# HKUST-Aerial-Robotics/Omni-swarm

Hardware: NVIDIA H100
Metric: keyframes/sec (SuperPoint+NetVLAD+match) (higher is better)
Workload: dtype f32

## Files before the change

omni-swarm_b200/csrc/kernels.cuh:

```cuda
#pragma once
#include "common.cuh"

namespace osb {

int db_scan_grid(int64_t n, int64_t* chunk_out);
osb_status db_search_device(const void* rows, int storage, int64_t n, const int64_t* n_dev, int dim, const float* q_dev,
                            int nq, int k, float* part_scores, int64_t* part_ids, unsigned int* done, float* scores_dev,
                            int64_t* ids_dev, cudaStream_t st);
osb_status db_rows_alloc(Resources& m, void** rows, size_t n, int storage);
osb_status db_rows_to_half(__half* dst, const float* src, size_t n, cudaStream_t st);
osb_status bf_match_device(int n_pairs, int max_n, int out_stride, const float* const* q, const int32_t* nq,
                           const float* const* t,
                           const int32_t* nt, float* dist_scratch, int32_t* qi, int32_t* ti, float* dout,
                           int32_t* n_out, int32_t* map_out, cudaStream_t st, int group = 0, size_t group_stride = 0);

enum Act { ACT_NONE = 0, ACT_RELU = 1, ACT_RELU6 = 2 };

struct ConvLayer {
  int cin = 0, cout = 0, cout_pad = 0, ks = 1;
  float* w = nullptr;
  float* b = nullptr;
};
osb_status conv_layer_upload(Resources& res, ConvLayer* L, const float* w_oihw, const float* bias, int cin, int cout, int ks);
osb_status upload_tap_major(Resources& res, float** dst, const float* w_oihw, int cout);

osb_status conv_forward(const ConvLayer& L, const float* x, float* y, int B, int H, int W, int out_cstride,
                        int act, cudaStream_t st);
osb_status conv_first_forward(const float* w_tap_cout , const float* bias, const float* lut,
                              const uint8_t* img, float* y, int B, int H, int W, int cout, int stride, int act,
                              cudaStream_t st);
osb_status maxpool2x2_forward(const float* x, float* y, int B, int H, int W, int C, cudaStream_t st);
osb_status dwconv3x3_forward(const float* w_tap_c, const float* bias, const float* x, float* y, int B, int H, int W,
                             int C, int stride, int act, cudaStream_t st);

osb_status sp_softmax_shuffle(const float* logits, int cstride, float* semi, int B, int Hc, int Wc, cudaStream_t st);
osb_status l2norm_cells(float* x, int64_t cells, int C, cudaStream_t st);

struct KeypointScratch {
  uint8_t* state = nullptr;
  uint8_t* surv = nullptr;
  int32_t* cand = nullptr;
  unsigned long long* skey = nullptr;
  unsigned long long* cmask = nullptr;
  bool write_surv = true;
  int32_t* counts = nullptr;
  float* cnorm = nullptr;
};
osb_status sp_keypoints(const float* semi, int B, int H, int W, float thres, int max_num, KeypointScratch& ks,
                        int32_t* n_kpts, float* kpts, float* conf, cudaStream_t st);
osb_status sp_descriptors(const float* desc_nhwc, int B, int H, int W, const int32_t* n_kpts, const float* kpts,
                          int max_num, const float* pca_compT , const float* pca_mean, float* cnorm, float* out,
                          cudaStream_t st);
osb_status nchw_to_nhwc(const float* in, float* out, int B, int C, int h, int w, cudaStream_t st);
osb_status nhwc_to_nchw(const float* in, float* out, int B, int C, int h, int w, cudaStream_t st);

osb_status stereo_lift_device(const float* kp_up, const float* kp_down, const int32_t* match, const int32_t* n_up,
                              const int32_t* n_down, int n_dirs, int max_n, const double* K, const double* pose_up,
                              const double* pose_down, double triangle_thres, int min_pts, float* pts3d, uint8_t* flag_up,
                              uint8_t* flag_down, cudaStream_t st, bool down_main = false);
osb_status depth_lift_device(const float* kp, const int32_t* n_kp, int n_dirs, int max_n, const uint16_t* depth_mm, int H,
                             int W, const double* K, const double* pose_cam, double near_thres, double far_thres,
                             int min_pts, float* pts3d, uint8_t* flag, cudaStream_t st);
osb_status homography_ransac_device(const float* src_dev, const float* dst_dev, const int32_t* n_dev, int n_pairs, int max_n,
                                    float thresh, uint32_t seed, uint8_t* mask_dev, int32_t* n_inl_dev, int32_t* winner_dev,
                                    cudaStream_t st, unsigned int* scratch );

constexpr int PNP_THREADS = 256;
constexpr int PNP_MAXN = 1024;
__global__ void __launch_bounds__(PNP_THREADS)
pnp_ransac_kernel(const float* __restrict__ pts3d, const float* __restrict__ pts2d, const int32_t* __restrict__ n_pts, int max_n,
                  const osb_pnp_params* __restrict__ params, uint8_t* __restrict__ mask_out, osb_pnp_result* __restrict__ results);

}
```

omni-swarm_b200/csrc/keyframe.cu:

```cuda
#include "superpoint.cuh"
#include "pose_algebra.cuh"
#include <atomic>

namespace osb {

struct DbDev {
  int64_t ntotal;
  int nframes;
};

struct FeFeedback {
  volatile long long seq_begin;
  volatile long long n_local, n_remote, charged;
  volatile long long seq_end;
};

struct DbView {
  DbDev* dev;
  int storage;
  void* rows;
  float* ldesc;
  float* kpts;
  int32_t* lflag;
  int32_t* nk;
// ... 722 lines not shown
  OSB_TRY(m.alloc(&g.g_mask, sk));
  OSB_TRY(m.alloc(&g.g_keys, 2 * (size_t)slots));
  OSB_CUDA(cudaMemsetAsync(g.g_keys, 0, 2 * (size_t)slots * sizeof(unsigned int), st));
  return OSB_OK;
}

extern "C" osb_status osb_frontend_create(osb_frontend** out, const osb_frontend_config* cfg, const float* sp_weights,
                                          size_t n_sp_weights, const float* pca_comp, const float* pca_mean,
                                          const float* nv_weights, size_t n_nv_weights) {
  OSB_REQUIRE(out && cfg && sp_weights && pca_comp && pca_mean && nv_weights, "null argument");
  OSB_REQUIRE(cfg->n_dirs >= 1 && cfg->n_dirs <= OSB_MAX_DIRS, "n_dirs must be 1..4");
  OSB_REQUIRE(cfg->max_num >= 1 && cfg->max_num <= OSB_MAX_KPTS, "max_num must be 1..200");
  OSB_REQUIRE(cfg->query_dir >= 0 && cfg->query_dir < cfg->n_dirs, "query_dir out of range");
  OSB_REQUIRE(cfg->db_capacity > 0 && cfg->db_capacity < (1 << 30), "bad db_capacity");
  OSB_REQUIRE(cfg->match_index_dist >= 1 && 5 + cfg->match_index_dist <= FE_KMAX, "bad match_index_dist");
  OSB_TRY(require_device());
  std::unique_ptr<osb_frontend> h(new osb_frontend());
  h->cfg = *cfg;
  h->device = current_device();
  const int nd = cfg->n_dirs, mn = cfg->max_num;
  Resources& m = h->res;
  OSB_TRY(m.stream(&h->stream));
  OSB_TRY(m.stream(&h->stream2));
  OSB_TRY(m.event(&h->ev_fork, cudaEventDisableTiming));
  OSB_TRY(m.event(&h->ev_join, cudaEventDisableTiming));
  OSB_TRY(m.event(&h->ev_ingest, cudaEventDisableTiming));
  OSB_TRY(m.host_alloc(&h->h_cnt, 2, cudaHostAllocDefault));
  OSB_TRY(m.host_alloc(&h->fb_host, 1, cudaHostAllocMapped));
  memset((void*)h->fb_host, 0, sizeof(FeFeedback));
  OSB_CUDA(cudaHostGetDevicePointer((void**)&h->fb_dev, (void*)h->fb_host, 0));
  OSB_TRY(h->sp.init(sp_weights, n_sp_weights, cfg->width, cfg->height, cfg->sp_thres, mn, pca_comp, pca_mean, 2 * nd));
  h->sp.ks.write_surv = false;
  if (cfg->zero_bottom_quarter) OSB_TRY(h->sp.band_init());
  OSB_TRY(h->nv.init(nv_weights, n_nv_weights, cfg->width, cfg->height, nd));
  OSB_TRY(dbstore_alloc(m, h->db[0], cfg->db_capacity, mn));
  OSB_TRY(dbstore_alloc(m, h->db[1], cfg->db_capacity, mn));
  const size_t HW = (size_t)cfg->width * cfg->height, dk = (size_t)OSB_MAX_DIRS * OSB_MAX_KPTS, dm = (size_t)OSB_MAX_DIRS * mn;
  OSB_TRY(m.alloc(&h->d_img, 2 * nd * HW));
  OSB_TRY(m.alloc(&h->d_st_pairs, 1));
  OSB_TRY(m.alloc(&h->d_q_pairs, 1));
  OSB_TRY(m.alloc(&h->d_st_qi, dm));
  OSB_TRY(m.alloc(&h->d_st_ti, dm));
  OSB_TRY(m.alloc(&h->d_st_map, dm));
  OSB_TRY(m.alloc(&h->d_st_n, OSB_MAX_DIRS));
  OSB_TRY(m.alloc(&h->d_st_dist, dm));
  OSB_TRY(m.alloc(&h->q1.dout, dk));
  OSB_TRY(fe_geo_alloc(m, h->q1, OSB_MAX_DIRS, 0));
  OSB_TRY(m.alloc(&h->d_dist_scratch, dm * mn));
  h->q1.pairs = fe_pair_view(h->d_q_pairs);
  h->q1.dist = h->d_dist_scratch;
  OSB_TRY(m.alloc(&h->d_assign, (size_t)h->max_records * OSB_MAX_DIRS));
  OSB_TRY(m.alloc(&h->d_cam_pose, 2 * OSB_MAX_DIRS * 7));
  OSB_TRY(m.alloc(&h->d_l3d, dm * 3));
  OSB_TRY(m.alloc(&h->d_lflag_up, dm));
  OSB_TRY(m.alloc(&h->d_lflag_down, dm));
  OSB_TRY(m.alloc(&h->d_record, 1));
  OSB_TRY(m.alloc(&h->d_result, 1));
  {
    FePairs st{};
    for (int d = 0; d < nd; ++d) {
      st.q[d] = h->sp.d_out + (size_t)d * mn * OSB_FEATURE_DESC_SIZE;
      st.t[d] = h->sp.d_out + (size_t)(nd + d) * mn * OSB_FEATURE_DESC_SIZE;
    }
    OSB_CUDA(cudaMemcpy(h->d_st_pairs, &st, sizeof(st), cudaMemcpyHostToDevice));
  }
  *out = h.release();
// ... 698 lines not shown
```

omni-swarm_b200/csrc/postproc.cu:

```cuda
#include "common.cuh"
#include "kernels.cuh"

namespace osb {

__global__ void sp_softmax_shuffle_kernel(const float* __restrict__ logits, int cstride, float* __restrict__ semi,
                                          int Hc, int Wc, int64_t cells) {
  const int64_t i = (int64_t)blockIdx.x * blockDim.x + threadIdx.x;
  if (i >= cells) return;
  const int cx = (int)(i % Wc);
  const int cy = (int)((i / Wc) % Hc);
  const int b = (int)(i / ((int64_t)Wc * Hc));
  const float* l = logits + (size_t)i * cstride;
  float v[65];
  float m = -INFINITY;
#pragma unroll
  for (int c = 0; c < 65; ++c) { v[c] = l[c]; m = fmaxf(m, v[c]); }
  float s = 0.f;
#pragma unroll
  for (int c = 0; c < 65; ++c) { v[c] = expf(v[c] - m); s += v[c]; }
  const int W = Wc * 8;
  float* out = semi + ((size_t)b * Hc * 8 + cy * 8) * W + cx * 8;
#pragma unroll
  for (int r = 0; r < 8; ++r) {
    float4 a = make_float4(v[r * 8 + 0] / s, v[r * 8 + 1] / s, v[r * 8 + 2] / s, v[r * 8 + 3] / s);
    float4 c = make_float4(v[r * 8 + 4] / s, v[r * 8 + 5] / s, v[r * 8 + 6] / s, v[r * 8 + 7] / s);
    reinterpret_cast<float4*>(out + (size_t)r * W)[0] = a;
    reinterpret_cast<float4*>(out + (size_t)r * W)[1] = c;
  }
}

osb_status sp_softmax_shuffle(const float* logits, int cstride, float* semi, int B, int Hc, int Wc, cudaStream_t st) {
  const int64_t cells = (int64_t)B * Hc * Wc;
  OSB_LAUNCH(sp_softmax_shuffle_kernel, (unsigned)cdiv64(cells, 128), 128, 0, st, logits, cstride, semi, Hc, Wc, cells);
  OSB_CHECK_LAUNCH();
  return OSB_OK;
}

__global__ void l2norm_cells_kernel(float* __restrict__ x, int64_t cells, int C) {
  const int64_t cell = ((int64_t)blockIdx.x * blockDim.x + threadIdx.x) >> 5;
  const int lane = threadIdx.x & 31;
  if (cell >= cells) return;
  float* p = x + (size_t)cell * C;
  float s = 0.f;
  for (int c = lane; c < C; c += 32) { const float v = p[c]; s = fmaf(v, v, s); }
  s = warp_sum(s);
  const float n = sqrtf(s);
  for (int c = lane; c < C; c += 32) p[c] = p[c] / n;
}

osb_status l2norm_cells(float* x, int64_t cells, int C, cudaStream_t st) {
  OSB_LAUNCH(l2norm_cells_kernel, (unsigned)cdiv64(cells * 32, 256), 256, 0, st, x, cells, C);
  OSB_CHECK_LAUNCH();
  return OSB_OK;
}

constexpr int KP_THREADS = 1024;
constexpr int KP_SORT_CAP = 8192;
constexpr int KP_RANK_CAP = 128;

__device__ __forceinline__ void load_state9(const uint8_t* __restrict__ state, int start, int HW, uint8_t (&out)[9]) {
  const int a0 = (start >> 3) << 3;
  const unsigned long long lo = (a0 >= 0 && a0 + 8 <= HW) ? __ldcg(reinterpret_cast<const unsigned long long*>(state + a0)) : 0ull;
  const unsigned long long hi = (a0 + 8 >= 0 && a0 + 16 <= HW) ? __ldcg(reinterpret_cast<const unsigned long long*>(state + a0 + 8)) : 0ull;
  const int sh = start - a0;
#pragma unroll
  for (int i = 0; i < 9; ++i) {
    const int bpos = i + sh;
    out[i] = (uint8_t)((bpos < 8 ? (lo >> (8 * bpos)) : (hi >> (8 * (bpos - 8)))) & 0xff);
  }
}

__device__ __forceinline__ void load_state9p(const uint8_t* __restrict__ state, int start, int HW, unsigned long long& w,
                                             unsigned& b8) {
  const int a0 = (start >> 3) << 3;
  const unsigned long long lo = (a0 >= 0 && a0 + 8 <= HW) ? __ldcg(reinterpret_cast<const unsigned long long*>(state + a0)) : 0ull;
  const unsigned long long hi = (a0 + 8 >= 0 && a0 + 16 <= HW) ? __ldcg(reinterpret_cast<const unsigned long long*>(state + a0 + 8)) : 0ull;
  const int sh = 8 * (start - a0);
  w = sh ? ((lo >> sh) | (hi << (64 - sh))) : lo;
  b8 = (unsigned)((hi >> sh) & 0xffull);
// ... 253 lines not shown
    counts[b * 8 + 6] = (int)(t_p3 - t_p2); counts[b * 8 + 7] = (int)(t_end - t_p3);
  }
}

osb_status sp_keypoints(const float* semi, int B, int H, int W, float thres, int max_num, KeypointScratch& ks,
                        int32_t* n_kpts, float* kpts, float* conf, cudaStream_t st) {
  OSB_REQUIRE((H * W) % 8 == 0, "H*W must be a multiple of 8");
  const size_t smem = (size_t)KP_SORT_CAP * sizeof(unsigned long long);
  OSB_SMEM_OPT_IN(sp_keypoints_kernel, smem);
  OSB_LAUNCH(sp_keypoints_kernel, B, KP_THREADS, smem, st, semi, H, W, thres, max_num, ks.state, ks.surv, ks.cand,
             ks.skey, ks.cmask, ks.write_surv ? 1 : 0, ks.counts, n_kpts, kpts, conf);
  OSB_CHECK_LAUNCH();
  return OSB_OK;
}

struct Taps { int x0, y0; float nw, ne, sw, se; };

__device__ __forceinline__ Taps bilinear_taps(float kx, float ky, int W, int H, int Wc, int Hc) {
  const float gx = __fsub_rn(__fdiv_rn(__fmul_rn(2.0f, kx), (float)W), 1.0f);
  const float gy = __fsub_rn(__fdiv_rn(__fmul_rn(2.0f, ky), (float)H), 1.0f);
  const float ix = __fdiv_rn(__fsub_rn(__fmul_rn(__fadd_rn(gx, 1.0f), (float)Wc), 1.0f), 2.0f);
  const float iy = __fdiv_rn(__fsub_rn(__fmul_rn(__fadd_rn(gy, 1.0f), (float)Hc), 1.0f), 2.0f);
  const float fx = floorf(ix), fy = floorf(iy);
  Taps t;
  t.x0 = (int)fx; t.y0 = (int)fy;
  const float ex = __fadd_rn(fx, 1.0f), ey = __fadd_rn(fy, 1.0f);
  t.nw = __fmul_rn(__fsub_rn(ex, ix), __fsub_rn(ey, iy));
  t.ne = __fmul_rn(__fsub_rn(ix, fx), __fsub_rn(ey, iy));
  t.sw = __fmul_rn(__fsub_rn(ex, ix), __fsub_rn(iy, fy));
  t.se = __fmul_rn(__fsub_rn(ix, fx), __fsub_rn(iy, fy));
  return t;
}

__device__ __forceinline__ float sample_channel(const float* __restrict__ d, const Taps& t, int Wc, int Hc, int ch) {
  float r = 0.f;
  const bool x0 = t.x0 >= 0 && t.x0 < Wc, x1 = t.x0 + 1 >= 0 && t.x0 + 1 < Wc;
  const bool y0 = t.y0 >= 0 && t.y0 < Hc, y1 = t.y0 + 1 >= 0 && t.y0 + 1 < Hc;
  if (y0 && x0) r = __fadd_rn(r, __fmul_rn(d[((size_t)t.y0 * Wc + t.x0) * 256 + ch], t.nw));
  if (y0 && x1) r = __fadd_rn(r, __fmul_rn(d[((size_t)t.y0 * Wc + t.x0 + 1) * 256 + ch], t.ne));
  if (y1 && x0) r = __fadd_rn(r, __fmul_rn(d[((size_t)(t.y0 + 1) * Wc + t.x0) * 256 + ch], t.sw));
  if (y1 && x1) r = __fadd_rn(r, __fmul_rn(d[((size_t)(t.y0 + 1) * Wc + t.x0 + 1) * 256 + ch], t.se));
  return r;
}

constexpr int DN_GROUPS = 16, DN_CH = 64;
__global__ void __launch_bounds__(DN_GROUPS * DN_CH)
sp_desc_norm_kernel(const float* __restrict__ desc, int H, int W, const int32_t* __restrict__ n_kpts,
                    const float* __restrict__ kpts, int max_num, float* __restrict__ cnorm) {
  __shared__ float part[DN_GROUPS][DN_CH];
  const int b = blockIdx.x, c = threadIdx.x % DN_CH, g = threadIdx.x / DN_CH;
  const int ch = blockIdx.y * DN_CH + c;
  const int Hc = H / 8, Wc = W / 8;
  const float* d = desc + (size_t)b * Hc * Wc * 256;
  const float* kp = kpts + (size_t)b * max_num * 2;
  const int N = n_kpts[b];
  float s = 0.f;
  for (int n = g; n < N; n += 2 * DN_GROUPS) {
    const int n2 = n + DN_GROUPS;
    const Taps t0 = bilinear_taps(kp[2 * n], kp[2 * n + 1], W, H, Wc, Hc);
    const Taps t1 = bilinear_taps(kp[2 * min(n2, N - 1)], kp[2 * min(n2, N - 1) + 1], W, H, Wc, Hc);
    const float v0 = sample_channel(d, t0, Wc, Hc, ch);
    const float v1 = sample_channel(d, t1, Wc, Hc, ch);
    s = fmaf(v0, v0, s);
    if (n2 < N) s = fmaf(v1, v1, s);
  }
  part[g][c] = s;
  __syncthreads();
  if (g == 0) {
    float t = 0.f;
#pragma unroll
    for (int i = 0; i < DN_GROUPS; ++i) t += part[i][c];
    cnorm[b * 256 + ch] = sqrtf(t);
  }
}

constexpr int DP_KP = 8;
__global__ void __launch_bounds__(256)
sp_desc_pca_kernel(const float* __restrict__ desc, int H, int W, const int32_t* __restrict__ n_kpts,
                   const float* __restrict__ kpts, int max_num, const float* __restrict__ cnorm,
                   const float* __restrict__ pca_compT, const float* __restrict__ pca_mean, float* __restrict__ out) {
  __shared__ float sv[DP_KP][256];
  const int b = blockIdx.y, n0 = blockIdx.x * DP_KP, tid = threadIdx.x;
  const int N = n_kpts[b];
  if (n0 >= N) return;
  const int Hc = H / 8, Wc = W / 8;
  const float* d = desc + (size_t)b * Hc * Wc * 256;
  const float cn = cnorm[b * 256 + tid], mu = pca_mean[tid];
#pragma unroll
  for (int i = 0; i < DP_KP; ++i) {
    const int n = n0 + i;
    float v = 0.f;
    if (n < N) {
      const Taps t = bilinear_taps(kpts[((size_t)b * max_num + n) * 2], kpts[((size_t)b * max_num + n) * 2 + 1], W, H, Wc, Hc);
      v = __fsub_rn(__fdiv_rn(sample_channel(d, t, Wc, Hc, tid), cn), mu);
    }
    sv[i][tid] = v;
  }
  __syncthreads();
  const int o = tid & 63, kq = tid >> 6;
  float a0 = 0.f, a1 = 0.f;
#pragma unroll 8
  for (int c = 0; c < 256; ++c) {
    const float w = __ldg(pca_compT + c * 64 + o);
    a0 = fmaf(sv[kq][c], w, a0);
    a1 = fmaf(sv[kq + 4][c], w, a1);
  }
  if (n0 + kq < N) out[((size_t)b * max_num + n0 + kq) * 64 + o] = a0;
  if (n0 + kq + 4 < N) out[((size_t)b * max_num + n0 + kq + 4) * 64 + o] = a1;
}

osb_status sp_descriptors(const float* desc_nhwc, int B, int H, int W, const int32_t* n_kpts, const float* kpts,
                          int max_num, const float* pca_compT, const float* pca_mean, float* cnorm, float* out,
                          cudaStream_t st) {
  OSB_LAUNCH(sp_desc_norm_kernel, dim3(B, 256 / DN_CH), DN_GROUPS * DN_CH, 0, st, desc_nhwc, H, W, n_kpts, kpts, max_num, cnorm);
  OSB_CHECK_LAUNCH();
  dim3 grid(cdiv(max_num, DP_KP), B);
  OSB_LAUNCH(sp_desc_pca_kernel, grid, 256, 0, st, desc_nhwc, H, W, n_kpts, kpts, max_num, cnorm, pca_compT, pca_mean, out);
  OSB_CHECK_LAUNCH();
  return OSB_OK;
}

__global__ void nchw_to_nhwc_kernel(const float* __restrict__ in, float* __restrict__ out, int C, int hw, int64_t total) {
  const int64_t i = (int64_t)blockIdx.x * blockDim.x + threadIdx.x;
  if (i >= total) return;
  const int c = (int)(i % C);
  const int64_t p = (i / C) % hw;
  const int64_t b = i / ((int64_t)C * hw);
  out[i] = in[(b * C + c) * hw + p];
}
__global__ void nhwc_to_nchw_kernel(const float* __restrict__ in, float* __restrict__ out, int C, int hw, int64_t total) {
  const int64_t i = (int64_t)blockIdx.x * blockDim.x + threadIdx.x;
  if (i >= total) return;
  const int64_t p = i % hw;
  const int c = (int)((i / hw) % C);
  const int64_t b = i / ((int64_t)C * hw);
  out[i] = in[(b * hw + p) * C + c];
}
osb_status nchw_to_nhwc(const float* in, float* out, int B, int C, int h, int w, cudaStream_t st) {
  const int64_t total = (int64_t)B * C * h * w;
  OSB_LAUNCH(nchw_to_nhwc_kernel, (unsigned)cdiv64(total, 256), 256, 0, st, in, out, C, h * w, total);
  OSB_CHECK_LAUNCH();
  return OSB_OK;
}
osb_status nhwc_to_nchw(const float* in, float* out, int B, int C, int h, int w, cudaStream_t st) {
  const int64_t total = (int64_t)B * C * h * w;
  OSB_LAUNCH(nhwc_to_nchw_kernel, (unsigned)cdiv64(total, 256), 256, 0, st, in, out, C, h * w, total);
  OSB_CHECK_LAUNCH();
  return OSB_OK;
}

// ... 2 lines not shown
```

omni-swarm_b200/csrc/superpoint.cu:

```cuda
#include "superpoint.cuh"
#include <stdlib.h>

namespace osb {

static const int SP_CIN[12] = {1, 64, 64, 64, 64, 128, 128, 128, 128, 256, 128, 256};
static const int SP_COUT[12] = {64, 64, 64, 64, 128, 128, 128, 128, 256, 65, 256, 256};
static const int SP_KS[12] = {3, 3, 3, 3, 3, 3, 3, 3, 3, 1, 3, 1};
constexpr float SP_ACT_SCALE = 16.f;
constexpr float SP_W_SCALE = 1024.f;
constexpr int SP_TRUNK = 8;
static const BandLayer SP_TRUNK_LAYERS[SP_TRUNK] = {{3, 0}, {3, 1}, {3, 0}, {3, 1}, {3, 0}, {3, 1}, {3, 0}, {3, 0}};
constexpr int SP_BAND_C = 128;

static void sp_band_geometry(int H, int W, int zero_row, TileRect* px, TileRect* tiles, TileRect* first_skip) {
  band_geometry(H, W, zero_row, SP_TRUNK_LAYERS, SP_TRUNK, px, tiles, first_skip);
}

static size_t band_offset(int prec, int layer, int plane) {
  const int p = prec == OSB_PRECISION_FP16 ? 1 : 0;
  return ((size_t)(p * SP_TRUNK + layer) * 2 + plane) * SP_BAND_C;
}

const __half* SuperPoint::band_const(int prec, int layer, int plane) const {
  return band_c + band_offset(prec, layer, plane);
}

osb_status SuperPoint::band_init() {
  if (!use_umma || band_c) return OSB_OK;
  TileRect px[SP_TRUNK], tiles[SP_TRUNK], skip;
  sp_band_geometry(H, W, 0, px, tiles, &skip);
  __half* c = nullptr;
  OSB_TRY(res.alloc(&c, (size_t)2 * SP_TRUNK * 2 * SP_BAND_C));
  OSB_CUDA(cudaMemsetAsync(d_img, 0, (size_t)H * W, stream));
  for (const int prec : {OSB_PRECISION_SPLIT_FP16, OSB_PRECISION_FP16}) {
    OSB_TRY(umma_first_forward(w1a, b1a, lut, d_img, in_hi[1], in_lo[1], 1, H, W, SP_ACT_SCALE, stream, prec));
    int h = H, w = W;
    for (int i = 1; i < SP_TRUNK; ++i) {
      const int pool = SP_TRUNK_LAYERS[i].pool;
      OSB_TRY(umma_conv_forward(UL[i], tmA[i], tmB[i], 1, h, w, SP_ACT_SCALE, in_hi[i + 1], in_lo[i + 1], nullptr,
                                SP_COUT[i], SP_COUT[i], SP_ACT_SCALE, 1, pool, stream, 0, prec));
      if (pool) { h /= 2; w /= 2; }
      if (px[i].empty()) continue;
      const size_t at = ((size_t)px[i].y0 * w + px[i].x0) * SP_COUT[i], bytes = SP_COUT[i] * sizeof(__half);
      OSB_CUDA(cudaMemcpyAsync(c + band_offset(prec, i, 0), in_hi[i + 1] + at, bytes, cudaMemcpyDeviceToDevice, stream));
      if (prec == OSB_PRECISION_SPLIT_FP16)
        OSB_CUDA(cudaMemcpyAsync(c + band_offset(prec, i, 1), in_lo[i + 1] + at, bytes, cudaMemcpyDeviceToDevice, stream));
    }
  }
  OSB_CUDA(cudaStreamSynchronize(stream));
  band_c = c;
  return OSB_OK;
}

size_t sp_expected_weights() {
  size_t n = 0;
  for (int i = 0; i < 12; ++i) n += (size_t)SP_COUT[i] * SP_CIN[i] * SP_KS[i] * SP_KS[i] + SP_COUT[i];
  return n;
}

osb_status SuperPoint::init(const float* weights, size_t n_weights, int width, int height, float thres_, int max_num_,
                            const float* pca_comp, const float* pca_mean, int max_batch_) {
  OSB_REQUIRE(weights && pca_comp && pca_mean, "null weights / pca");
  OSB_REQUIRE(n_weights == sp_expected_weights(), "weight blob has the wrong length (expected 1300865 floats)");
  OSB_REQUIRE(width > 0 && height > 0 && width % 8 == 0 && height % 8 == 0, "width/height must be multiples of 8");
  OSB_REQUIRE(max_num_ > 0 && max_num_ <= 8192 && max_batch_ > 0, "bad max_num / max_batch");
  W = width; H = height; thres = thres_; max_num = max_num_; max_batch = max_batch_;
  Hc = H / 8; Wc = W / 8;
  OSB_TRY(res.stream(&stream));
  {
    int least = 0, greatest = 0;
    OSB_CUDA(cudaDeviceGetStreamPriorityRange(&least, &greatest));
    OSB_TRY(res.stream(&kp_stream, greatest));
  }
  OSB_TRY(res.event(&ev_semi, cudaEventDisableTiming));
  OSB_TRY(res.event(&ev_kp, cudaEventDisableTiming));
  if (const char* e = getenv("OSB_SP_OVERLAP")) overlap_kp = atoi(e) != 0;
  if (const char* e = getenv("OSB_SP_FUSED_SOFTMAX")) fused_softmax = atoi(e) != 0;
  const float* p = weights;
  {
    std::vector<float> w9(9 * 64);
    for (int o = 0; o < 64; ++o)
      for (int t = 0; t < 9; ++t) w9[t * 64 + o] = p[o * 9 + t];
    OSB_TRY(res.upload(&w1a, w9.data(), 9 * 64));
    OSB_TRY(res.upload(&b1a, p + 64 * 9, 64));
    p += 64 * 9 + 64;
  }
  {
    const char* e = getenv("OSB_SP_CONV");
    use_umma = !(e && strcmp(e, "ffma") == 0);
  }
  for (int i = 1; i < 12; ++i) {
    const size_t nw = (size_t)SP_COUT[i] * SP_CIN[i] * SP_KS[i] * SP_KS[i];
    OSB_TRY(conv_layer_upload(res, &L[i], p, p + nw, SP_CIN[i], SP_COUT[i], SP_KS[i]));
    if (use_umma) OSB_TRY(umma_layer_upload(res, &UL[i], p, p + nw, SP_CIN[i], SP_COUT[i], SP_KS[i], SP_W_SCALE));
    p += nw + SP_COUT[i];
  }
  {
    std::vector<float> l(256);
    const float alpha = (float)(1.0 / 255.0);
    for (int v = 0; v < 256; ++v) l[v] = (float)v * alpha;
    OSB_TRY(res.upload(&lut, l.data(), 256));
  }
  {
    std::vector<float> ct(256 * 64);
    for (int o = 0; o < 64; ++o)
      for (int c = 0; c < 256; ++c) ct[c * 64 + o] = pca_comp[o * 256 + c];
    OSB_TRY(res.upload(&pca_compT, ct.data(), 256 * 64));
    OSB_TRY(res.upload(&pca_mean_d, pca_mean, 256));
  }
  const size_t B = max_batch, HW = (size_t)H * W;
  OSB_TRY(res.alloc(&d_img, B * HW));
  OSB_TRY(res.alloc(&actA, B * HW * 64));
  OSB_TRY(res.alloc(&actB, B * HW * 64));
  OSB_TRY(res.alloc(&d_logits, B * Hc * Wc * 80));
  if (use_umma) {
    const int in_buf[12] = {-1, 0, 1, 0, 1, 0, 1, 0, 1, 0, 1, 0};
    const int in_div[12] = {0, 1, 2, 2, 4, 4, 8, 8, 8, 8, 8, 8};
    for (int i = 1; i < 12; ++i) {
      const int h = H / in_div[i], w = W / in_div[i], c = SP_CIN[i];
      __half* base = reinterpret_cast<__half*>(in_buf[i] == 0 ? actA : actB);
      in_hi[i] = base;
      in_lo[i] = base + (size_t)max_batch * h * w * c;
      OSB_TRY(umma_act_maps(&tmA[i], &tmB[i], in_hi[i], in_lo[i], max_batch, h, w, c, SP_KS[i]));
    }
  }
  OSB_TRY(res.alloc(&d_semi, B * HW));
  OSB_TRY(res.alloc(&d_desc, B * Hc * Wc * 256));
// ... 25 lines not shown
    if (banded && i < SP_TRUNK)
      band = ConvBand{band_tiles[i], band_const(precision, i, 0), band_const(precision, i, 1)};
    return umma_conv_forward(UL[i], tmA[i], tmB[i], B, h, w, SA, in_hi[out_layer], in_lo[out_layer], nullptr,
                             SP_COUT[i], SP_COUT[i], SA, 1, pool, st, 0, precision, &band);
  };
  OSB_TRY(umma_first_forward(w1a, b1a, lut, img_dev, in_hi[1], in_lo[1], B, H, W, SA, st, precision,
                             banded ? first_skip : TileRect{}));
  mark(st);
  OSB_TRY(conv(1, H, W, 2, 1));
  mark(st);
  OSB_TRY(conv(2, H / 2, W / 2, 3, 0));
  mark(st);
  OSB_TRY(conv(3, H / 2, W / 2, 4, 1));
  mark(st);
  OSB_TRY(conv(4, H / 4, W / 4, 5, 0));
  mark(st);
  OSB_TRY(conv(5, H / 4, W / 4, 6, 1));
  mark(st);
  OSB_TRY(conv(6, Hc, Wc, 7, 0));
  mark(st);
  OSB_TRY(conv(7, Hc, Wc, 8, 0));
  mark(st);
  OSB_TRY(conv(8, Hc, Wc, 9, 0));
  mark(st);
  if (fused_softmax) {
    OSB_TRY(umma_conv_softmax_forward(UL[9], tmA[9], tmB[9], B, Hc, Wc, SA, d_semi, st, 0, precision));
    mark(st);
  } else {
    OSB_TRY(umma_conv_forward(UL[9], tmA[9], tmB[9], B, Hc, Wc, SA, nullptr, nullptr, d_logits, 80, 80, 1.f, 0, 0, st, 0,
                              precision));
    mark(st);
    OSB_TRY(sp_softmax_shuffle(d_logits, 80, d_semi, B, Hc, Wc, st));
  }
  const bool fork = kp && overlap_kp && !layer_prof && kp_stream;
  int head_ctas = 0;
  if (fork) {
    OSB_CUDA(cudaEventRecord(ev_semi, st));
    OSB_CUDA(cudaStreamWaitEvent(kp_stream, ev_semi, 0));
    OSB_TRY(keypoints(B, *kp, kp_stream));
    OSB_CUDA(cudaEventRecord(ev_kp, kp_stream));
    head_ctas = std::max(1, persistent_ctas() - B);
  }
  OSB_TRY(umma_conv_forward(UL[10], tmA[10], tmB[10], B, Hc, Wc, SA, in_hi[11], in_lo[11], nullptr, SP_COUT[10], SP_COUT[10],
                            SA, 1, 0, st, head_ctas, precision));
  mark(st);
  OSB_TRY(umma_conv_forward(UL[11], tmA[11], tmB[11], B, Hc, Wc, SA, nullptr, nullptr, d_desc, 256, 256, 1.f, 0, 0, st,
                            head_ctas, precision));
  mark(st);
  OSB_TRY(l2norm_cells(d_desc, (int64_t)B * Hc * Wc, 256, st));
  if (fork) OSB_CUDA(cudaStreamWaitEvent(st, ev_kp, 0));
  else if (kp) OSB_TRY(keypoints(B, *kp, st));
  return OSB_OK;
}

osb_status SuperPoint::network(const uint8_t* img_dev, int B, cudaStream_t st, const KpJob* kp, int zero_row) {
  if (use_umma) return network_umma(img_dev, B, st, kp, zero_row);
  OSB_TRY(conv_first_forward(w1a, b1a, lut, img_dev, actA, B, H, W, 64, 1, ACT_RELU, st));
  OSB_TRY(conv_forward(L[1], actA, actB, B, H, W, 64, ACT_RELU, st));
  OSB_TRY(maxpool2x2_forward(actB, actA, B, H, W, 64, st));
  OSB_TRY(conv_forward(L[2], actA, actB, B, H / 2, W / 2, 64, ACT_RELU, st));
  OSB_TRY(conv_forward(L[3], actB, actA, B, H / 2, W / 2, 64, ACT_RELU, st));
  OSB_TRY(maxpool2x2_forward(actA, actB, B, H / 2, W / 2, 64, st));
  OSB_TRY(conv_forward(L[4], actB, actA, B, H / 4, W / 4, 128, ACT_RELU, st));
  OSB_TRY(conv_forward(L[5], actA, actB, B, H / 4, W / 4, 128, ACT_RELU, st));
  OSB_TRY(maxpool2x2_forward(actB, actA, B, H / 4, W / 4, 128, st));
  OSB_TRY(conv_forward(L[6], actA, actB, B, Hc, Wc, 128, ACT_RELU, st));
  OSB_TRY(conv_forward(L[7], actB, actA, B, Hc, Wc, 128, ACT_RELU, st));
  OSB_TRY(conv_forward(L[8], actA, actB, B, Hc, Wc, 256, ACT_RELU, st));
  OSB_TRY(conv_forward(L[9], actB, d_logits, B, Hc, Wc, 72, ACT_NONE, st));
  OSB_TRY(conv_forward(L[10], actA, actB, B, Hc, Wc, 256, ACT_RELU, st));
  OSB_TRY(conv_forward(L[11], actB, d_desc, B, Hc, Wc, 256, ACT_NONE, st));
  OSB_TRY(l2norm_cells(d_desc, (int64_t)B * Hc * Wc, 256, st));
  OSB_TRY(sp_softmax_shuffle(d_logits, 72, d_semi, B, Hc, Wc, st));
  if (kp) OSB_TRY(keypoints(B, *kp, st));
  return OSB_OK;
}

osb_status SuperPoint::keypoints(int B, const KpJob& kp, cudaStream_t st) {
  return sp_keypoints(d_semi, B, H, W, thres, max_num, ks, kp.nk, kp.kpts, kp.conf, st);
}

osb_status SuperPoint::descriptors(int B, const KpJob& kp, float* out, cudaStream_t st) {
  return sp_descriptors(d_desc, B, H, W, kp.nk, kp.kpts, max_num, pca_compT, pca_mean_d, ks.cnorm, out, st);
}

osb_status SuperPoint::postprocess(int B, int32_t* nk, float* kpts, float* conf, float* out, cudaStream_t st) {
  const KpJob kp{nk, kpts, conf};
  osb_status s = keypoints(B, kp, st);
  if (s != OSB_OK) return s;
  return descriptors(B, kp, out, st);
}

osb_status SuperPoint::forward(const uint8_t* img_dev, int B, int32_t* nk, float* kpts, float* conf, float* out,
                               cudaStream_t st) {
  OSB_REQUIRE(B > 0 && B <= max_batch, "batch out of range");
  const KpJob kp{nk, kpts, conf};
  osb_status s = network(img_dev, B, st, &kp);
  if (s != OSB_OK) return s;
  last_batch = B;
  return descriptors(B, kp, out, st);
}

osb_status SuperPoint::infer_dev(const uint8_t* img_dev, int B, int32_t* nk, float* kpts, float* out, cudaStream_t st) {
  return forward(img_dev, B, nk, kpts, d_conf, out, st);
}

}

using namespace osb;

struct osb_superpoint {
  int device = 0;
  SuperPoint sp;
  std::mutex mu;
};

extern "C" osb_status osb_superpoint_create(osb_superpoint** out, const float* weights, size_t n_weights, int width,
                                            int height, float thres, int max_num, const float* pca_comp,
                                            const float* pca_mean, int max_batch) {
// ... 145 lines not shown
```

omni-swarm_b200/csrc/superpoint.cuh:

```cuda
#pragma once
#include "common.cuh"
#include "kernels.cuh"
#include "conv_umma.cuh"

namespace osb {

size_t sp_expected_weights();
size_t nv_expected_weights();

inline osb_status umma_set_precision(bool use_umma, int* precision, int p) {
  OSB_REQUIRE(p == OSB_PRECISION_SPLIT_FP16 || p == OSB_PRECISION_FP16,
              "precision must be OSB_PRECISION_SPLIT_FP16 or OSB_PRECISION_FP16");
  OSB_REQUIRE(use_umma || p == OSB_PRECISION_SPLIT_FP16,
              "plain fp16 needs the tensor-core convolutions (the handle was created under OSB_SP_CONV=ffma)");
  *precision = p;
  return OSB_OK;
}

struct SuperPoint {
  Resources res;
  int W = 0, H = 0, Wc = 0, Hc = 0, max_num = 0, max_batch = 0, last_batch = 0;
  float thres = 0.f;
  cudaStream_t stream = nullptr;
  float *w1a = nullptr, *b1a = nullptr, *lut = nullptr, *pca_compT = nullptr, *pca_mean_d = nullptr;
  ConvLayer L[12];
  uint8_t* d_img = nullptr;
  float *actA = nullptr, *actB = nullptr, *d_logits = nullptr, *d_semi = nullptr, *d_desc = nullptr;
  KeypointScratch ks;
  int32_t* d_nk = nullptr;
  float *d_kpts = nullptr, *d_conf = nullptr, *d_out = nullptr;

  bool use_umma = true;
  int precision = OSB_PRECISION_SPLIT_FP16;
  UmmaLayer UL[12];
  CUtensorMap tmA[12], tmB[12];
  __half *in_hi[12] = {}, *in_lo[12] = {};
  __half* band_c = nullptr;
  const __half* band_const(int prec, int layer, int plane) const;
  osb_status band_init();
  bool layer_prof = false;
  cudaEvent_t lev[20] = {};
  int n_lev = 0;
  void mark(cudaStream_t st) { if (layer_prof && n_lev < 20) { if (!lev[n_lev]) res.event(&lev[n_lev]); cudaEventRecord(lev[n_lev++], st); } }

  osb_status init(const float* weights, size_t n_weights, int width, int height, float thres, int max_num,
                  const float* pca_comp, const float* pca_mean, int max_batch);
  osb_status set_precision(int p) { return umma_set_precision(use_umma, &precision, p); }
  struct KpJob { int32_t* nk; float* kpts; float* conf; };
  cudaStream_t kp_stream = nullptr;
  cudaEvent_t ev_semi = nullptr, ev_kp = nullptr;
  bool overlap_kp = true;
  bool fused_softmax = true;
  osb_status network(const uint8_t* img_dev, int B, cudaStream_t st, const KpJob* kp = nullptr, int zero_row = -1);
  osb_status network_umma(const uint8_t* img_dev, int B, cudaStream_t st, const KpJob* kp, int zero_row);
  osb_status keypoints(int B, const KpJob& kp, cudaStream_t st);
  osb_status descriptors(int B, const KpJob& kp, float* out, cudaStream_t st);
  osb_status forward(const uint8_t* img_dev, int B, int32_t* nk, float* kpts, float* conf, float* out, cudaStream_t st);
  osb_status postprocess(int B, int32_t* nk, float* kpts, float* conf, float* out, cudaStream_t st);
  osb_status infer_dev(const uint8_t* img_dev, int B, int32_t* nk, float* kpts, float* out, cudaStream_t st);
};

struct NetVLAD {
  Resources res;
  int W = 0, H = 0, max_batch = 0;
  cudaStream_t stream = nullptr;
  float *w0 = nullptr, *b0 = nullptr, *lut = nullptr, *pw0_kc = nullptr, *pw0_b = nullptr;
  struct Block { float *dw = nullptr, *dwb = nullptr; ConvLayer pw; int cin = 0, cout = 0, stride = 1; } blk[7];
  ConvLayer proj, assign;
  float* centroids = nullptr;
  uint8_t* d_img = nullptr;
  float *actA = nullptr, *actB = nullptr, *d_assign = nullptr, *d_out = nullptr;
  float *d_mu = nullptr, *d_part = nullptr, *d_psum = nullptr;
  bool use_umma = true;
  int precision = OSB_PRECISION_SPLIT_FP16;
  UmmaLayer upw[7], uproj;
  CUtensorMap tmA[8], tmB[8];
  __half *pl_hi[8] = {}, *pl_lo[8] = {};
  __half* planes = nullptr;

  osb_status init(const float* weights, size_t n_weights, int width, int height, int max_batch);
  osb_status set_precision(int p) { return umma_set_precision(use_umma, &precision, p); }
// ... 5 lines not shown
```

Baseline: 424.1.

## Compute SuperPoint descriptor head only on cells touched by keypoints

Adds a sparse descriptor head. After keypoints are found, the cells used by bilinear sampling are marked and compacted, and their 3x3 neighbourhoods are gathered into an im2col buffer. The two descriptor convolutions then run as tensor-core GEMMs on those rows only, instead of over the full feature map. The descriptor norm and PCA kernels read through a slot indirection with per-cell L2 norms. This cuts descriptor-head FLOPs and memory traffic, but it serialises keypoint extraction before the head, so the keypoint/head overlap is lost, and it adds gather and extra-kernel overhead.

Result: faster. 438.6, median of 6 (+3.4%).

```diff
diff --git a/omni-swarm_b200/csrc/kernels.cuh b/omni-swarm_b200/csrc/kernels.cuh
--- a/omni-swarm_b200/csrc/kernels.cuh
+++ b/omni-swarm_b200/csrc/kernels.cuh
@@ -50,6 +50,9 @@
                         int32_t* n_kpts, float* kpts, float* conf, cudaStream_t st);
 osb_status sp_descriptors(const float* desc_nhwc, int B, int H, int W, const int32_t* n_kpts, const float* kpts,
                           int max_num, const float* pca_compT , const float* pca_mean, float* cnorm, float* out,
+                          cudaStream_t st, const int32_t* slot = nullptr, int seg = 0, float* cell_n = nullptr);
+osb_status sp_cell_gather(int B, int H, int W, const int32_t* n_kpts, const float* kpts, int max_num, int seg, int32_t* slot,
+                          const __half* x_hi, const __half* x_lo, __half* col_hi, __half* col_lo, bool fp16,
                           cudaStream_t st);
 osb_status nchw_to_nhwc(const float* in, float* out, int B, int C, int h, int w, cudaStream_t st);
 osb_status nhwc_to_nchw(const float* in, float* out, int B, int C, int h, int w, cudaStream_t st);
diff --git a/omni-swarm_b200/csrc/keyframe.cu b/omni-swarm_b200/csrc/keyframe.cu
--- a/omni-swarm_b200/csrc/keyframe.cu
+++ b/omni-swarm_b200/csrc/keyframe.cu
@@ -778,6 +778,7 @@
   OSB_TRY(h->sp.init(sp_weights, n_sp_weights, cfg->width, cfg->height, cfg->sp_thres, mn, pca_comp, pca_mean, 2 * nd));
   h->sp.ks.write_surv = false;
   if (cfg->zero_bottom_quarter) OSB_TRY(h->sp.band_init());
+  OSB_TRY(h->sp.sparse_init());
   OSB_TRY(h->nv.init(nv_weights, n_nv_weights, cfg->width, cfg->height, nd));
   OSB_TRY(dbstore_alloc(m, h->db[0], cfg->db_capacity, mn));
   OSB_TRY(dbstore_alloc(m, h->db[1], cfg->db_capacity, mn));
diff --git a/omni-swarm_b200/csrc/postproc.cu b/omni-swarm_b200/csrc/postproc.cu
--- a/omni-swarm_b200/csrc/postproc.cu
+++ b/omni-swarm_b200/csrc/postproc.cu
@@ -36,15 +36,19 @@
   return OSB_OK;
 }
 
+__device__ __forceinline__ float cell_norm(const float* p, int C, int lane) {
+  float s = 0.f;
+  for (int c = lane; c < C; c += 32) { const float v = p[c]; s = fmaf(v, v, s); }
+  s = warp_sum(s);
+  return sqrtf(s);
+}
+
 __global__ void l2norm_cells_kernel(float* __restrict__ x, int64_t cells, int C) {
   const int64_t cell = ((int64_t)blockIdx.x * blockDim.x + threadIdx.x) >> 5;
   const int lane = threadIdx.x & 31;
   if (cell >= cells) return;
   float* p = x + (size_t)cell * C;
-  float s = 0.f;
-  for (int c = lane; c < C; c += 32) { const float v = p[c]; s = fmaf(v, v, s); }
-  s = warp_sum(s);
-  const float n = sqrtf(s);
+  const float n = cell_norm(p, C, lane);
   for (int c = lane; c < C; c += 32) p[c] = p[c] / n;
 }
 
@@ -364,26 +368,123 @@
   return t;
 }
 
-__device__ __forceinline__ float sample_channel(const float* __restrict__ d, const Taps& t, int Wc, int Hc, int ch) {
+template <bool SLOT = false>
+__device__ __forceinline__ float sample_channel(const float* __restrict__ d, const int32_t* __restrict__ slot,
+                                                const float* nrm, int row0, const Taps& t, int Wc, int Hc, int ch) {
+  auto at = [&](int y, int x) {
+    if constexpr (SLOT) {
+      const int row = slot[y * Wc + x];
+      return d[(size_t)row * 256 + ch] / nrm[row - row0];
+    } else {
+      return d[((size_t)y * Wc + x) * 256 + ch];
+    }
+  };
   float r = 0.f;
   const bool x0 = t.x0 >= 0 && t.x0 < Wc, x1 = t.x0 + 1 >= 0 && t.x0 + 1 < Wc;
   const bool y0 = t.y0 >= 0 && t.y0 < Hc, y1 = t.y0 + 1 >= 0 && t.y0 + 1 < Hc;
-  if (y0 && x0) r = __fadd_rn(r, __fmul_rn(d[((size_t)t.y0 * Wc + t.x0) * 256 + ch], t.nw));
-  if (y0 && x1) r = __fadd_rn(r, __fmul_rn(d[((size_t)t.y0 * Wc + t.x0 + 1) * 256 + ch], t.ne));
-  if (y1 && x0) r = __fadd_rn(r, __fmul_rn(d[((size_t)(t.y0 + 1) * Wc + t.x0) * 256 + ch], t.sw));
-  if (y1 && x1) r = __fadd_rn(r, __fmul_rn(d[((size_t)(t.y0 + 1) * Wc + t.x0 + 1) * 256 + ch], t.se));
+  if (y0 && x0) r = __fadd_rn(r, __fmul_rn(at(t.y0, t.x0), t.nw));
+  if (y0 && x1) r = __fadd_rn(r, __fmul_rn(at(t.y0, t.x0 + 1), t.ne));
+  if (y1 && x0) r = __fadd_rn(r, __fmul_rn(at(t.y0 + 1, t.x0), t.sw));
+  if (y1 && x1) r = __fadd_rn(r, __fmul_rn(at(t.y0 + 1, t.x0 + 1), t.se));
   return r;
 }
 
+constexpr int CL_THREADS = KP_THREADS;
+constexpr int CL_SPLIT = 16;
+template <bool FP16>
+__global__ void __launch_bounds__(CL_THREADS)
+sp_cell_gather_kernel(int H, int W, const int32_t* __restrict__ n_kpts, const float* __restrict__ kpts, int max_num, int seg,
+                      int32_t* __restrict__ slot, const __half* __restrict__ x_hi, const __half* __restrict__ x_lo,
+                      __half* __restrict__ col_hi, __half* __restrict__ col_lo) {
+  extern __shared__ int32_t list[];
+  __shared__ int wsum[32], total;
+  const int b = blockIdx.x, tid = threadIdx.x, Hc = H / 8, Wc = W / 8, cells = Hc * Wc;
+  uint8_t* mark = reinterpret_cast<uint8_t*>(list + seg);
+  for (int c = tid; c < cells; c += CL_THREADS) mark[c] = 0;
+  __syncthreads();
+  const int N = n_kpts[b];
+  for (int n = tid; n < N; n += CL_THREADS) {
+    const Taps t = bilinear_taps(kpts[((size_t)b * max_num + n) * 2], kpts[((size_t)b * max_num + n) * 2 + 1], W, H, Wc, Hc);
+    for (int dy = 0; dy < 2; ++dy)
+      for (int dx = 0; dx < 2; ++dx) {
+        const int y = t.y0 + dy, x = t.x0 + dx;
+        if (y >= 0 && y < Hc && x >= 0 && x < Wc) mark[y * Wc + x] = 1;
+      }
+  }
+  __syncthreads();
+  const int per = (cells + CL_THREADS - 1) / CL_THREADS, c0 = tid * per, c1 = min(c0 + per, cells);
+  int cnt = 0;
+  for (int c = c0; c < c1; ++c) cnt += mark[c];
+  int rank = block_exclusive_scan(cnt, wsum, &total);
+  const bool writer = blockIdx.y == 0;
+  for (int c = c0; c < c1; ++c) {
+    if (mark[c]) {
+      if (writer) slot[(size_t)b * cells + c] = b * seg + rank;
+      list[rank++] = c;
+    } else if (writer) {
+      slot[(size_t)b * cells + c] = -1;
+    }
+  }
+  for (int r = total + tid; r < seg; r += CL_THREADS) list[r] = -1;
+  __syncthreads();
+  for (int e = blockIdx.y * CL_THREADS + tid; e < seg * 144; e += CL_SPLIT * CL_THREADS) {
+    const int i = e / 144, r = e % 144, tap = r / 16, j = r % 16, ky = tap / 3, kx = tap % 3, s = j / 8;
+    const int c = list[i];
+    uint4 h = make_uint4(0, 0, 0, 0), l = h;
+    if (c >= 0) {
+      const int y = c / Wc + ky - 1, xx = c % Wc + kx - 1;
+      if (y >= 0 && y < Hc && xx >= 0 && xx < Wc) {
+        const size_t src = (((size_t)b * Hc + y) * Wc + xx) * 128 + j * 8;
+        h = *reinterpret_cast<const uint4*>(x_hi + src);
+        if constexpr (!FP16) l = *reinterpret_cast<const uint4*>(x_lo + src);
+      }
+    }
+    const size_t dst = ((size_t)b * seg + i) * 1152 + ((kx * 2 + s) * 3 + ky) * 64 + (j % 8) * 8;
+    *reinterpret_cast<uint4*>(col_hi + dst) = h;
+    if constexpr (!FP16) *reinterpret_cast<uint4*>(col_lo + dst) = l;
+  }
+}
+
+osb_status sp_cell_gather(int B, int H, int W, const int32_t* n_kpts, const float* kpts, int max_num, int seg, int32_t* slot,
+                          const __half* x_hi, const __half* x_lo, __half* col_hi, __half* col_lo, bool fp16,
+                          cudaStream_t st) {
+  const int smem = seg * 4 + (H / 8) * (W / 8);
+  OSB_REQUIRE(smem <= 48 * 1024, "sparse descriptor head: too many cells per image");
+  const dim3 grid(B, CL_SPLIT);
+  if (fp16)
+    OSB_LAUNCH(sp_cell_gather_kernel<true>, grid, CL_THREADS, smem, st, H, W, n_kpts, kpts, max_num, seg, slot, x_hi, x_lo,
+               col_hi, col_lo);
+  else
+    OSB_LAUNCH(sp_cell_gather_kernel<false>, grid, CL_THREADS, smem, st, H, W, n_kpts, kpts, max_num, seg, slot, x_hi, x_lo,
+               col_hi, col_lo);
+  OSB_CHECK_LAUNCH();
+  return OSB_OK;
+}
+
 constexpr int DN_GROUPS = 16, DN_CH = 64;
+template <bool SLOT = false>
 __global__ void __launch_bounds__(DN_GROUPS * DN_CH)
-sp_desc_norm_kernel(const float* __restrict__ desc, int H, int W, const int32_t* __restrict__ n_kpts,
-                    const float* __restrict__ kpts, int max_num, float* __restrict__ cnorm) {
+sp_desc_norm_kernel(const float* __restrict__ desc, const int32_t* __restrict__ slot, int seg, float* __restrict__ cell_n,
+                    int H, int W, const int32_t* __restrict__ n_kpts, const float* __restrict__ kpts, int max_num,
+                    float* __restrict__ cnorm) {
   __shared__ float part[DN_GROUPS][DN_CH];
+  extern __shared__ float nrm[];
   const int b = blockIdx.x, c = threadIdx.x % DN_CH, g = threadIdx.x / DN_CH;
   const int ch = blockIdx.y * DN_CH + c;
   const int Hc = H / 8, Wc = W / 8;
-  const float* d = desc + (size_t)b * Hc * Wc * 256;
+  const float* d = SLOT ? desc : desc + (size_t)b * Hc * Wc * 256;
+  const int32_t* sl = SLOT ? slot + (size_t)b * Hc * Wc : nullptr;
+  if constexpr (SLOT) {
+    const int lane = threadIdx.x & 31;
+    for (int r = threadIdx.x >> 5; r < seg; r += DN_GROUPS * DN_CH / 32) {
+      const float n = cell_norm(desc + ((size_t)b * seg + r) * 256, 256, lane);
+      if (lane == 0) {
+        nrm[r] = n;
+        if (blockIdx.y == 0) cell_n[(size_t)b * seg + r] = n;
+      }
+    }
+    __syncthreads();
+  }
   const float* kp = kpts + (size_t)b * max_num * 2;
   const int N = n_kpts[b];
   float s = 0.f;
@@ -391,8 +492,8 @@
     const int n2 = n + DN_GROUPS;
     const Taps t0 = bilinear_taps(kp[2 * n], kp[2 * n + 1], W, H, Wc, Hc);
     const Taps t1 = bilinear_taps(kp[2 * min(n2, N - 1)], kp[2 * min(n2, N - 1) + 1], W, H, Wc, Hc);
-    const float v0 = sample_channel(d, t0, Wc, Hc, ch);
-    const float v1 = sample_channel(d, t1, Wc, Hc, ch);
+    const float v0 = sample_channel<SLOT>(d, sl, nrm, b * seg, t0, Wc, Hc, ch);
+    const float v1 = sample_channel<SLOT>(d, sl, nrm, b * seg, t1, Wc, Hc, ch);
     s = fmaf(v0, v0, s);
     if (n2 < N) s = fmaf(v1, v1, s);
   }
@@ -407,8 +508,10 @@
 }
 
 constexpr int DP_KP = 8;
+template <bool SLOT = false>
 __global__ void __launch_bounds__(256)
-sp_desc_pca_kernel(const float* __restrict__ desc, int H, int W, const int32_t* __restrict__ n_kpts,
+sp_desc_pca_kernel(const float* __restrict__ desc, const int32_t* __restrict__ slot, const float* __restrict__ cell_n,
+                   int H, int W, const int32_t* __restrict__ n_kpts,
                    const float* __restrict__ kpts, int max_num, const float* __restrict__ cnorm,
                    const float* __restrict__ pca_compT, const float* __restrict__ pca_mean, float* __restrict__ out) {
   __shared__ float sv[DP_KP][256];
@@ -416,7 +519,8 @@
   const int N = n_kpts[b];
   if (n0 >= N) return;
   const int Hc = H / 8, Wc = W / 8;
-  const float* d = desc + (size_t)b * Hc * Wc * 256;
+  const float* d = SLOT ? desc : desc + (size_t)b * Hc * Wc * 256;
+  const int32_t* sl = SLOT ? slot + (size_t)b * Hc * Wc : nullptr;
   const float cn = cnorm[b * 256 + tid], mu = pca_mean[tid];
 #pragma unroll
   for (int i = 0; i < DP_KP; ++i) {
@@ -424,7 +528,7 @@
     float v = 0.f;
     if (n < N) {
       const Taps t = bilinear_taps(kpts[((size_t)b * max_num + n) * 2], kpts[((size_t)b * max_num + n) * 2 + 1], W, H, Wc, Hc);
-      v = __fsub_rn(__fdiv_rn(sample_channel(d, t, Wc, Hc, tid), cn), mu);
+      v = __fsub_rn(__fdiv_rn(sample_channel<SLOT>(d, sl, cell_n, 0, t, Wc, Hc, tid), cn), mu);
     }
     sv[i][tid] = v;
   }
@@ -443,11 +547,22 @@
 
 osb_status sp_descriptors(const float* desc_nhwc, int B, int H, int W, const int32_t* n_kpts, const float* kpts,
                           int max_num, const float* pca_compT, const float* pca_mean, float* cnorm, float* out,
-                          cudaStream_t st) {
-  OSB_LAUNCH(sp_desc_norm_kernel, dim3(B, 256 / DN_CH), DN_GROUPS * DN_CH, 0, st, desc_nhwc, H, W, n_kpts, kpts, max_num, cnorm);
-  OSB_CHECK_LAUNCH();
-  dim3 grid(cdiv(max_num, DP_KP), B);
-  OSB_LAUNCH(sp_desc_pca_kernel, grid, 256, 0, st, desc_nhwc, H, W, n_kpts, kpts, max_num, cnorm, pca_compT, pca_mean, out);
+                          cudaStream_t st, const int32_t* slot, int seg, float* cell_n) {
+  const dim3 gn(B, 256 / DN_CH), gp(cdiv(max_num, DP_KP), B);
+  if (slot) {
+    OSB_REQUIRE(seg * 4 <= 48 * 1024 && cell_n, "sparse descriptor head: too many rows per image");
+    OSB_LAUNCH(sp_desc_norm_kernel<true>, gn, DN_GROUPS * DN_CH, seg * 4, st, desc_nhwc, slot, seg, cell_n, H, W, n_kpts,
+               kpts, max_num, cnorm);
+    OSB_CHECK_LAUNCH();
+    OSB_LAUNCH(sp_desc_pca_kernel<true>, gp, 256, 0, st, desc_nhwc, slot, cell_n, H, W, n_kpts, kpts, max_num, cnorm,
+               pca_compT, pca_mean, out);
+  } else {
+    OSB_LAUNCH(sp_desc_norm_kernel<false>, gn, DN_GROUPS * DN_CH, 0, st, desc_nhwc, slot, 0, cell_n, H, W, n_kpts, kpts,
+               max_num, cnorm);
+    OSB_CHECK_LAUNCH();
+    OSB_LAUNCH(sp_desc_pca_kernel<false>, gp, 256, 0, st, desc_nhwc, slot, cell_n, H, W, n_kpts, kpts, max_num, cnorm,
+               pca_compT, pca_mean, out);
+  }
   OSB_CHECK_LAUNCH();
   return OSB_OK;
 }
diff --git a/omni-swarm_b200/csrc/superpoint.cu b/omni-swarm_b200/csrc/superpoint.cu
--- a/omni-swarm_b200/csrc/superpoint.cu
+++ b/omni-swarm_b200/csrc/superpoint.cu
@@ -52,6 +52,36 @@
   return OSB_OK;
 }
 
+osb_status SuperPoint::sparse_init() {
+  if (const char* e = getenv("OSB_SP_SPARSE_HEAD")) if (atoi(e) == 0) return OSB_OK;
+  if (!use_umma || sparse_head) return OSB_OK;
+  seg = cdiv(std::min(4 * max_num, Hc * Wc), 128) * 128;
+  const size_t rows = (size_t)max_batch * seg;
+  OSB_TRY(res.alloc(&cell_slot, (size_t)max_batch * Hc * Wc));
+  OSB_TRY(res.alloc(&cell_n, rows));
+  OSB_TRY(res.alloc(&col_hi, rows * 1152));
+  OSB_TRY(res.alloc(&col_lo, rows * 1152));
+  OSB_TRY(res.alloc(&da_hi, rows * 256));
+  OSB_TRY(res.alloc(&da_lo, rows * 256));
+  OSB_TRY(res.alloc(&desc_c, rows * 256));
+  const int tiles = (int)(rows / 128);
+  OSB_TRY(umma_act_maps(&tm_col[0], &tm_col[1], col_hi, col_lo, tiles, 8, 16, 1152, 1));
+  OSB_TRY(umma_act_maps(&tm_da[0], &tm_da[1], da_hi, da_lo, tiles, 8, 16, 256, 1));
+  sparse_head = true;
+  return OSB_OK;
+}
+
+osb_status SuperPoint::sparse_desc_head(int B, const KpJob& kp, cudaStream_t st) {
+  const float SA = SP_ACT_SCALE;
+  const int tiles = B * seg / 128;
+  OSB_TRY(sp_cell_gather(B, H, W, kp.nk, kp.kpts, max_num, seg, cell_slot, in_hi[10], in_lo[10], col_hi, col_lo,
+                         precision == OSB_PRECISION_FP16, st));
+  OSB_TRY(umma_conv_forward(UDa_col, tm_col[0], tm_col[1], tiles, 8, 16, SA, da_hi, da_lo, nullptr, 256, 256, SA, 1, 0, st,
+                            0, precision));
+  return umma_conv_forward(UL[11], tm_da[0], tm_da[1], tiles, 8, 16, SA, nullptr, nullptr, desc_c, 256, 256, 1.f, 0, 0, st,
+                           0, precision);
+}
+
 size_t sp_expected_weights() {
   size_t n = 0;
   for (int i = 0; i < 12; ++i) n += (size_t)SP_COUT[i] * SP_CIN[i] * SP_KS[i] * SP_KS[i] + SP_COUT[i];
@@ -93,6 +123,16 @@
     const size_t nw = (size_t)SP_COUT[i] * SP_CIN[i] * SP_KS[i] * SP_KS[i];
     OSB_TRY(conv_layer_upload(res, &L[i], p, p + nw, SP_CIN[i], SP_COUT[i], SP_KS[i]));
     if (use_umma) OSB_TRY(umma_layer_upload(res, &UL[i], p, p + nw, SP_CIN[i], SP_COUT[i], SP_KS[i], SP_W_SCALE));
+    if (use_umma && i == 10) {
+      std::vector<float> wc((size_t)256 * 1152);
+      for (int o = 0; o < 256; ++o)
+        for (int c = 0; c < 128; ++c)
+          for (int t = 0; t < 9; ++t) {
+            const int ky = t / 3, kx = t % 3, slab = (kx * 2 + c / 64) * 3 + ky;
+            wc[(size_t)o * 1152 + slab * 64 + c % 64] = p[((size_t)o * 128 + c) * 9 + t];
+          }
+      OSB_TRY(umma_layer_upload(res, &UDa_col, wc.data(), p + nw, 1152, 256, 1, SP_W_SCALE));
+    }
     p += nw + SP_COUT[i];
   }
   {
@@ -184,6 +224,11 @@
     mark(st);
     OSB_TRY(sp_softmax_shuffle(d_logits, 80, d_semi, B, Hc, Wc, st));
   }
+  sparse_ran = sparse_head && kp && !layer_prof;
+  if (sparse_ran) {
+    OSB_TRY(keypoints(B, *kp, st));
+    return sparse_desc_head(B, *kp, st);
+  }
   const bool fork = kp && overlap_kp && !layer_prof && kp_stream;
   int head_ctas = 0;
   if (fork) {
@@ -206,6 +251,7 @@
 }
 
 osb_status SuperPoint::network(const uint8_t* img_dev, int B, cudaStream_t st, const KpJob* kp, int zero_row) {
+  sparse_ran = false;
   if (use_umma) return network_umma(img_dev, B, st, kp, zero_row);
   OSB_TRY(conv_first_forward(w1a, b1a, lut, img_dev, actA, B, H, W, 64, 1, ACT_RELU, st));
   OSB_TRY(conv_forward(L[1], actA, actB, B, H, W, 64, ACT_RELU, st));
@@ -233,10 +279,14 @@
 }
 
 osb_status SuperPoint::descriptors(int B, const KpJob& kp, float* out, cudaStream_t st) {
+  if (sparse_ran)
+    return sp_descriptors(desc_c, B, H, W, kp.nk, kp.kpts, max_num, pca_compT, pca_mean_d, ks.cnorm, out, st, cell_slot, seg,
+                          cell_n);
   return sp_descriptors(d_desc, B, H, W, kp.nk, kp.kpts, max_num, pca_compT, pca_mean_d, ks.cnorm, out, st);
 }
 
 osb_status SuperPoint::postprocess(int B, int32_t* nk, float* kpts, float* conf, float* out, cudaStream_t st) {
+  sparse_ran = false;
   const KpJob kp{nk, kpts, conf};
   osb_status s = keypoints(B, kp, st);
   if (s != OSB_OK) return s;
diff --git a/omni-swarm_b200/csrc/superpoint.cuh b/omni-swarm_b200/csrc/superpoint.cuh
--- a/omni-swarm_b200/csrc/superpoint.cuh
+++ b/omni-swarm_b200/csrc/superpoint.cuh
@@ -38,6 +38,14 @@
   __half* band_c = nullptr;
   const __half* band_const(int prec, int layer, int plane) const;
   osb_status band_init();
+  UmmaLayer UDa_col;
+  bool sparse_head = false, sparse_ran = false;
+  int seg = 0;
+  int32_t* cell_slot = nullptr;
+  __half *col_hi = nullptr, *col_lo = nullptr, *da_hi = nullptr, *da_lo = nullptr;
+  float *desc_c = nullptr, *cell_n = nullptr;
+  CUtensorMap tm_col[2], tm_da[2];
+  osb_status sparse_init();
   bool layer_prof = false;
   cudaEvent_t lev[20] = {};
   int n_lev = 0;
@@ -47,6 +55,7 @@
                   const float* pca_comp, const float* pca_mean, int max_batch);
   osb_status set_precision(int p) { return umma_set_precision(use_umma, &precision, p); }
   struct KpJob { int32_t* nk; float* kpts; float* conf; };
+  osb_status sparse_desc_head(int B, const KpJob& kp, cudaStream_t st);
   cudaStream_t kp_stream = nullptr;
   cudaEvent_t ev_semi = nullptr, ev_kp = nullptr;
   bool overlap_kp = true;
```
